# XuZhang1211/PVPUFormer

Measured on AMD Instinct MI355X. Metric: 448x448 images/sec fwd+bwd, ViT-B VPUFormer, higher is better.
Workload: dtype bf16

## Files before the change

include/vpu_hip.h:

```cpp
#ifndef VPU_HIP_H
#define VPU_HIP_H
#include <stdint.h>

#ifdef __cplusplus
extern "C" {
#endif

#define VPU_BF16 0
#define VPU_F32 1

#define VPU_EPI_BIAS 1
#define VPU_EPI_PREACT 2
#define VPU_EPI_GELU 4
#define VPU_EPI_RELU 8
#define VPU_EPI_DGELU 16
#define VPU_EPI_DRELU 32
#define VPU_EPI_RESID 64
#define VPU_EPI_AFFINE 128
#define VPU_EPI_ACCUM 256
#define VPU_EPI_OUT_F32 512
#define VPU_EPI_SAVE_DGELU 1024
#define VPU_EPI_MULAUX 2048

typedef struct vpu_gemm_desc {
// ... 186 lines not shown
    const uint8_t* valid;
    int32_t H, W, r0, r1, c0, c1, mirror, n_obj;
} vpu_box_row;
int vpu_box_prompts_batched(const vpu_box_row* rows, int32_t n_rows, const float* points, int32_t n_batch, int32_t S_h,
                            int32_t S_w, float pred_thresh, uint8_t* masks, int32_t* counts, int32_t* roots, int32_t* slots,
                            int32_t* table, int32_t kmax, int32_t* boxes, int32_t* flag, void* stream);
#define VPU_CROPS_MAX_TILES_AXIS 64
int vpu_crops_gather(const float* in, float* out, const int32_t* y_offsets, const int32_t* x_offsets, int32_t ny, int32_t nx,
                     int32_t C, int32_t H, int32_t W, int32_t ch, int32_t cw, void* stream);
int vpu_crops_blend(const float* probs, float* out, const int32_t* y_offsets, const int32_t* x_offsets, int32_t ny, int32_t nx,
                    int32_t H, int32_t W, int32_t ch, int32_t cw, void* stream);
int vpu_cc_roots(const uint8_t* mask, int32_t* roots, int32_t B, int32_t H, int32_t W, void* stream);
int vpu_cc_table(const int32_t* roots, int32_t* slots, int32_t* table, int32_t kmax, int32_t B, int32_t H, int32_t W,
                 void* stream);

int vpu_disk_maps(const float* points, const int32_t* boxes, float* out, int32_t B, int32_t n, int32_t H, int32_t W,
                  float radius, void* stream);

int vpu_patch_im2col(const float* image4, const float* disks, void* cols, int32_t B, int32_t H, int32_t W, int32_t P,
                     int32_t win_tokens, int32_t dtype, void* stream);
int vpu_patch_im2col_prenorm(const float* image4, const float* disks, void* cols, int32_t B, int32_t H, int32_t W, int32_t P,
                             int32_t win_tokens, int32_t dtype, void* stream);
int vpu_patch_im2col_floor(const float* image4, const float* disks, void* cols, int32_t B, int32_t H, int32_t W, int32_t P,
                           int32_t wside, int32_t prenorm, int32_t dtype, void* stream);
int vpu_window_permute(const void* x, void* y, int32_t B, int32_t g, int32_t wg, int32_t C, int32_t dir, int32_t dtype,
                       void* stream);

int vpu_pixel_shuffle2(const void* in, void* out, const float* bias, int32_t B, int32_t h, int32_t w, int32_t C,
                       int32_t dir, int32_t dtype, void* stream);
int vpu_space_to_depth2_crop(const void* in, void* out, int32_t B, int32_t g, int32_t C, int32_t dir, int32_t dtype,
                             void* stream);
int vpu_pixel_shuffle2_gn_stats(const void* in, void* out, const float* bias, double* stats, int32_t B, int32_t h, int32_t w,
                                int32_t C, int32_t dtype, void* stream);
int vpu_groupnorm_apply(const void* x, const float* w, const float* b, void* y, float* mean, float* rstd, const double* stats,
                        int32_t B, int64_t HW, int32_t C, float eps, int32_t gelu, int32_t dtype, void* stream);
int vpu_pixel_unshuffle2_nblk(int32_t C);
int vpu_pixel_unshuffle2_sums(const void* in, void* out, float* part, int32_t B, int32_t h, int32_t w, int32_t C,
                              int32_t dtype, void* stream);
int vpu_groupnorm_nchunk(void);
int vpu_groupnorm_fwd(const void* x, const float* w, const float* b, void* y, float* mean, float* rstd, double* stats,
                      int32_t B, int64_t HW, int32_t C, float eps, int32_t gelu, int32_t dtype, void* stream);
int vpu_groupnorm_bwd(const void* dy, const void* x, const float* w, const float* b, const float* mean,
                      const float* rstd, void* dx, float* part, double* stats, int32_t B, int64_t HW, int32_t C,
                      int32_t gelu, int32_t dtype, void* stream);
int vpu_bilinear_cl_fwd(const void* in, int32_t ld_in, void* out, int32_t ld_out, int32_t B, int32_t h, int32_t w,
                        int32_t H, int32_t W, int32_t C, int32_t dtype, void* stream);
int vpu_bilinear_cl_bwd(const void* dout, int32_t ld_out, void* din, int32_t ld_in, int32_t B, int32_t h, int32_t w,
                        int32_t H, int32_t W, int32_t C, int32_t dtype, void* stream);
int vpu_upsum_relu(void* io, const void* const* z, const int32_t* h, const int32_t* w, int32_t n, int32_t B, int32_t H,
                   int32_t W, int32_t C, int32_t dtype, void* stream);
int vpu_head_grad_fused(const void* dfn, const void* y, const float* inv, const float* dout, const void* x, const float* w,
                        const float* mask, void* dx, float* part, float* part_b, int64_t rows, int64_t HW, int32_t C,
                        int32_t dtype, void* stream);
int vpu_gate_stats(const void* Q, const void* Kt, float* cg, int32_t* argq, float* sg, int32_t* argc, int32_t B,
                   int32_t nq, int32_t N, int32_t C, int32_t dtype, void* stream);
int vpu_gate_apply(const void* x, const float* cg, const float* sg, void* out, int32_t B, int32_t N, int32_t C,
                   int32_t dtype, void* stream);
int vpu_gate_bwd(const void* dout, const void* x, const float* cg, const int32_t* argq, const float* sg,
                 const int32_t* argc, void* dx, int32_t accum, void* dQ, void* dK, float* part, int32_t B, int32_t nq,
                 int32_t N, int32_t C, int32_t dtype, void* stream);
int vpu_gate_fwd_n(const void* const* Q, const void* const* K, const void* x, void* const* out, float* cg, int32_t* argq,
                   float* sg, int32_t* argc, int32_t n, int32_t B, int32_t nq, int32_t N, int32_t C, int32_t dtype, void* stream);
int vpu_gate_bwd_n(const void* const* dout, const void* x, const float* cg, const int32_t* argq, const float* sg,
                   const int32_t* argc, void* dx, int32_t accum, void* const* dQ, void* const* dK, float* part, int32_t n,
                   int32_t B, int32_t nq, int32_t N, int32_t C, int32_t dtype, void* stream);
int vpu_convseg_fwd(const void* x, const float* w, const float* bias, const float* mask, float* out, int64_t rows,
                    int64_t HW, int32_t C, int32_t dtype, void* stream);
int vpu_convseg_bwd_nblk(int64_t rows);
int vpu_convseg_bwd(const float* dout, const void* x, const float* w, const float* mask, void* dx, int32_t accum,
                    float* part, float* part_b, int64_t rows, int64_t HW, int32_t C, int32_t dtype, void* stream);

int vpu_upsample_ac_fwd(const float* in, float* out, int64_t planes, int32_t h, int32_t w, int32_t H, int32_t W,
                        void* stream);
int vpu_upsample_ac_bwd(const float* dout, float* din, int64_t planes, int32_t h, int32_t w, int32_t H, int32_t W,
                        void* stream);
int vpu_p2cl_fwd_bwd(const float* prob, const float* gt, const int32_t* slot_mask_idx, const float* override_masks,
                     float* loss_part, float* dprob, float grad_scale, int32_t B, int32_t S, int32_t H, int32_t W,
                     void* stream);
int vpu_p2cl_up_nband(int32_t h, int32_t w);
int vpu_p2cl_up_fwd_bwd(const float* sim_low, const float* gt, const int32_t* slot_mask_idx, const float* override_masks,
                        float* loss_part, float* dsim_low, float grad_scale, int32_t B, int32_t S, int32_t h, int32_t w,
                        int32_t H, int32_t W, void* stream);
int vpu_nfl_dice_scratch_doubles(int32_t B);
int vpu_nfl_dice_fwd_bwd(const float* logits, const float* gt, double* sums, float* out, float* dlogits, float w_nfl,
                         float w_dice, int32_t B, int64_t HW, void* stream);

int vpu_loss_finalize(const float* out, const float* part, int32_t B, int32_t npart, double inv_count, float w_nfl,
                      float w_dice, float w_pcl, float iter_weight, float* res, void* stream);

int vpu_adam_step(float* p, const float* g, float* m, float* v, void* shadow_bf16, int64_t n, float lr, float beta1,
                  float beta2, float eps, float weight_decay, int32_t step, float grad_scale, void* stream);
int vpu_adam_step_groups(float* p, const float* g, float* m, float* v, void* shadow_bf16, int64_t n,
                         const int64_t* seg_end, const float* seg_lr, const float* seg_wd, int32_t nseg, float beta1,
                         float beta2, float eps, int32_t decoupled_wd, int32_t step, float grad_scale, void* stream);
int vpu_adam_step_hyper(float* p, const float* g, float* m, float* v, void* shadow_bf16, int64_t n, const float* hyper,
                        const int64_t* seg_end, const float* seg_scale, const float* seg_wd, int32_t nseg, float beta1,
                        float beta2, float eps, float weight_decay, int32_t decoupled_wd, void* stream);


#ifdef __cplusplus
}
#endif
#endif
```

pvpuformer_amd/_lib.py:

```python
import ctypes as C
import os

_HERE = os.path.dirname(os.path.abspath(__file__))
LIB_PATH = os.path.join(_HERE, os.environ.get("VPU_LIB_FILE") or
                        ("libvpu_hip_diag.so" if os.environ.get("VPU_LIB_DIAG", "0") == "1" else "libvpu_hip.so"))

BF16, F32 = 0, 1

EPI_BIAS, EPI_PREACT, EPI_GELU, EPI_RELU, EPI_DGELU, EPI_DRELU = 1, 2, 4, 8, 16, 32
EPI_RESID, EPI_AFFINE, EPI_ACCUM, EPI_OUT_F32 = 64, 128, 256, 512
EPI_SAVE_DGELU, EPI_MULAUX = 1024, 2048


class GemmDesc(C.Structure):
    _fields_ = [
        ("A", C.c_void_p), ("B", C.c_void_p), ("C", C.c_void_p), ("bias", C.c_void_p), ("resid", C.c_void_p),
        ("aux", C.c_void_p), ("preact", C.c_void_p),
        ("M", C.c_int32), ("N", C.c_int32), ("K", C.c_int32),
        ("lda", C.c_int32), ("ldb", C.c_int32), ("ldc", C.c_int32), ("ldr", C.c_int32), ("ldaux", C.c_int32),
        ("batch", C.c_int32), ("inner", C.c_int32),
        ("sAo", C.c_int64), ("sAi", C.c_int64), ("sBo", C.c_int64), ("sBi", C.c_int64),
        ("sCo", C.c_int64), ("sCi", C.c_int64), ("sRo", C.c_int64), ("sRi", C.c_int64),
        ("transA", C.c_int32), ("transB", C.c_int32), ("dtype", C.c_int32), ("flags", C.c_int32),
        ("resid_period", C.c_int32),
# ... 74 lines not shown
    "vpu_add_bcast": [_P, _P, _P, _L, _L, _I, _P],
    "vpu_add4": [_P, _P, _P, _P, _P, _L, _I, _P],
    "vpu_cast2d": [_P, _I, _L, _P, _I, _L, _L, _I, _I, _P],
    "vpu_cast2d_batched": [C.POINTER(CastJob), _I, _P],
    "vpu_fanout_add": [_P, C.POINTER(C.c_void_p), C.POINTER(C.c_int32), _I, _L, _I, _P],
    "vpu_dropout_mask": [_P, _I, _F, C.c_uint64, _P, _P],
    "vpu_fill_f32": [_P, _F, _L, _P],
    "vpu_fill_ranges_f32": [_P, C.POINTER(C.c_int64), C.POINTER(C.c_int64), _I, _F, _P],
    "vpu_debug_spin": [_P, _I, _L, _P],
    "vpu_debug_gemm_times": [_P],
    "vpu_sigmoid_to_channel": [_P, _P, _I, _L, _I, _I, _P],
    "vpu_act_bwd": [_P, _L, _P, _L, _P, _L, _L, _I, _I, _I, _P],
    "vpu_pue_encode": [_P, _P, _P, _P, _P, _I, _I, _I, _I, _I, _I, _P],
    "vpu_cc_roots": [_P, _P, _I, _I, _I, _P],
    "vpu_cc_table": [_P, _P, _P, _I, _I, _I, _I, _P],
    "vpu_edt": [_P, _P, _P, _I, _I, _I, _I, _P],
    "vpu_chamfer5": [_P, _P, _P, _I, _I, _I, _I, _P],
    "vpu_pue_scribble_rows": [_P, _P, _P, _P, _I, _I, _I, _I, _I, _I, _P],
    "vpu_draw_polyline": [_P, _P, _I, _I, _I, _I, _P],
    "vpu_pue_encode_rows": [_P, _P, _P, _P, _P, _P, _P, _I, _I, _I, _I, _I, _I, _P],
    "vpu_draw_prompt_rows": [_P, _P, _P, _P, _P, _I, _I, _I, _I, _I, _P],
    "vpu_mask_bbox": [_P, _F, _P, _I, _P, _I, _I, _I, _P],
    "vpu_masked_argmax": [_P, _P, _P, _I, _I, _I, _P],
    "vpu_error_masks": [_P, _P, _P, _P, _I, _I, _P],
    "vpu_roi_resize_batched": [_P, _I, _P, _I, _I, _I, _I, _P],
    "vpu_roi_paste_batched": [_P, _I, _P, _I, _I, _F, _F, _I, _P],
    "vpu_session_paste_batched": [_P, _I, _P, _I, _I, _F, _F, _I, _I, _P],
    "vpu_annot_compose_batched": [_P, _I, _F, _I, _P],
    "vpu_label_extract": [_P, _P, _P, _I, _I, _I, _P],
    "vpu_runs_count_batched": [_P, _P, _I, _P, _L, _P, _P],
    "vpu_runs_write_batched": [_P, _P, _I, _P, _L, _P, _I, _P],
    "vpu_runs_decode_batched": [_P, _P, _I, _P],
    "vpu_click_keys_batched": [_P, _I, _P, _P, _P, _I, _I, _I, _P],
    "vpu_box_prompts_batched": [_P, _I, _P, _I, _I, _I, _F, _P, _P, _P, _P, _P, _I, _P, _P, _P],
    "vpu_crops_gather": [_P, _P, _P, _P, _I, _I, _I, _I, _I, _I, _I, _P],
    "vpu_crops_blend": [_P, _P, _P, _P, _I, _I, _I, _I, _I, _I, _P],
    "vpu_disk_maps": [_P, _P, _P, _I, _I, _I, _I, _F, _P],
    "vpu_patch_im2col": [_P, _P, _P, _I, _I, _I, _I, _I, _I, _P],
    "vpu_patch_im2col_prenorm": [_P, _P, _P, _I, _I, _I, _I, _I, _I, _P],
    "vpu_patch_im2col_floor": [_P, _P, _P, _I, _I, _I, _I, _I, _I, _I, _P],
    "vpu_window_permute": [_P, _P, _I, _I, _I, _I, _I, _I, _P],
    "vpu_space_to_depth2_crop": [_P, _P, _I, _I, _I, _I, _I, _P],
    "vpu_pixel_shuffle2": [_P, _P, _P, _I, _I, _I, _I, _I, _I, _P],
    "vpu_pixel_shuffle2_gn_stats": [_P, _P, _P, _P, _I, _I, _I, _I, _I, _P],
    "vpu_groupnorm_apply": [_P, _P, _P, _P, _P, _P, _P, _I, _L, _I, _F, _I, _I, _P],
    "vpu_pixel_unshuffle2_nblk": [_I],
    "vpu_pixel_unshuffle2_sums": [_P, _P, _P, _I, _I, _I, _I, _I, _P],
    "vpu_groupnorm_nchunk": [],
    "vpu_groupnorm_fwd": [_P, _P, _P, _P, _P, _P, _P, _I, _L, _I, _F, _I, _I, _P],
    "vpu_groupnorm_bwd": [_P, _P, _P, _P, _P, _P, _P, _P, _P, _I, _L, _I, _I, _I, _P],
    "vpu_bilinear_cl_fwd": [_P, _I, _P, _I, _I, _I, _I, _I, _I, _I, _I, _P],
    "vpu_bilinear_cl_bwd": [_P, _I, _P, _I, _I, _I, _I, _I, _I, _I, _I, _P],
    "vpu_head_grad_fused": [_P, _P, _P, _P, _P, _P, _P, _P, _P, _P, _L, _L, _I, _I, _P],
    "vpu_upsum_relu": [_P, C.POINTER(C.c_void_p), C.POINTER(C.c_int32), C.POINTER(C.c_int32), _I, _I, _I, _I, _I, _I, _P],
    "vpu_gate_stats": [_P, _P, _P, _P, _P, _P, _I, _I, _I, _I, _I, _P],
    "vpu_gate_apply": [_P, _P, _P, _P, _I, _I, _I, _I, _P],
    "vpu_gate_bwd": [_P, _P, _P, _P, _P, _P, _P, _I, _P, _P, _P, _I, _I, _I, _I, _I, _P],
    "vpu_gate_fwd_n": [C.POINTER(C.c_void_p), C.POINTER(C.c_void_p), _P, C.POINTER(C.c_void_p), _P, _P, _P, _P, _I, _I, _I, _I, _I, _I, _P],
    "vpu_gate_bwd_n": [C.POINTER(C.c_void_p), _P, _P, _P, _P, _P, _P, _I, C.POINTER(C.c_void_p), C.POINTER(C.c_void_p), _P, _I, _I, _I,
                       _I, _I, _I, _P],
    "vpu_convseg_fwd": [_P, _P, _P, _P, _P, _L, _L, _I, _I, _P],
    "vpu_convseg_bwd_nblk": [_L],
    "vpu_convseg_bwd": [_P, _P, _P, _P, _P, _I, _P, _P, _L, _L, _I, _I, _P],
    "vpu_upsample_ac_fwd": [_P, _P, _L, _I, _I, _I, _I, _P],
    "vpu_upsample_ac_bwd": [_P, _P, _L, _I, _I, _I, _I, _P],
    "vpu_p2cl_fwd_bwd": [_P, _P, _P, _P, _P, _P, _F, _I, _I, _I, _I, _P],
    "vpu_p2cl_up_nband": [_I, _I],
    "vpu_p2cl_up_fwd_bwd": [_P, _P, _P, _P, _P, _P, _F, _I, _I, _I, _I, _I, _I, _P],
    "vpu_nfl_dice_scratch_doubles": [_I],
    "vpu_nfl_dice_fwd_bwd": [_P, _P, _P, _P, _P, _F, _F, _I, _L, _P],
    "vpu_loss_finalize": [_P, _P, _I, _I, C.c_double, _F, _F, _F, _F, _P, _P],
    "vpu_adam_step": [_P, _P, _P, _P, _P, _L, _F, _F, _F, _F, _F, _I, _F, _P],
    "vpu_adam_step_groups": [_P, _P, _P, _P, _P, _L, _P, _P, _P, _I, _F, _F, _F, _I, _I, _F, _P],
    "vpu_adam_step_hyper": [_P, _P, _P, _P, _P, _L, _P, _P, _P, _P, _I, _F, _F, _F, _F, _I, _P],
    "vpu_gemm_set_option": [C.c_char_p, _I],
    "vpu_gemm_get_option": [C.c_char_p, C.POINTER(C.c_int32)],
    "vpu_gemm_last_kernel": [],
    "vpu_attn_last_kernel": [],
    "vpu_attn_set_option": [C.c_char_p, _I],
    "vpu_gemm_grouped": [C.POINTER(GemmDesc), _I, _P],
    "vpu_last_error": [],
    "vpu_abi_version": [],
}
_RET = {"vpu_last_error": C.c_char_p, "vpu_gemm_last_kernel": C.c_char_p, "vpu_attn_last_kernel": C.c_char_p}

_lib = None


class VpuError(RuntimeError):
    pass


def load():
    global _lib
    if _lib is not None:
        return _lib
    if not os.path.exists(LIB_PATH):
        raise VpuError(f"{LIB_PATH} not found: build it with pvpuformer_amd/csrc/build.sh "
                       f"(or `python -c 'import __graft_entry__ as g; g.build()'`). There is no CPU fallback.")
    import torch
    lib = C.CDLL(LIB_PATH)
    for name, argtypes in SIGNATURES.items():
        fn = getattr(lib, name)
        fn.argtypes = argtypes
        fn.restype = _RET.get(name, C.c_int)
    _lib = lib
# ... 10 lines not shown
```

pvpuformer_amd/engine.py:

```python
import contextlib
import math
import os
from collections import OrderedDict
from types import SimpleNamespace

import numpy as np
import torch

from . import ops
from ._lib import (BF16, F32, EPI_BIAS, EPI_PREACT, EPI_GELU, EPI_RELU, EPI_DGELU, EPI_DRELU, EPI_RESID, EPI_AFFINE,
                   EPI_ACCUM, EPI_OUT_F32, EPI_SAVE_DGELU, EPI_MULAUX)


class Tape:
    __slots__ = ("fns", "out_grads", "done", "sim_low", "lane")

    def __init__(self):
        self.fns = []
        self.out_grads = [None, None, None]
        self.done = False
        self.sim_low = None
        self.lane = None

    def append(self, fn):
# ... 58 lines not shown


def check_square(H, W):
    if H != W:
        raise ValueError(f"input {H}x{W}: only square inputs are supported (the reference's neck takes h = w = sqrt(HW))")


class Engine:
    def __init__(self, cfg, dtype="bf16", device="cuda"):
        self.cfg = dict(cfg)
        self.dt = BF16 if dtype in ("bf16", BF16) else F32
        self.td = torch.bfloat16 if self.dt == BF16 else torch.float32
        self.dev = torch.device(device)
        c = self.cfg
        self.D, self.P, self.img = c["embed_dim"], c["patch"], c["img"]
        self.g, _, self.wside = window_geometry(self.img, self.P)
        self.NT = self.g * self.g
        self.heads = c["num_heads"]
        self.depth = c["depth"]
        self.group = 6 if self.depth == 12 else self.depth // 4
        self.nmax = c["num_max_points"]
        self.E = 2 * self.img + 3
        self.Epad = _rup(self.E, 8)
        self.C = c["head_channels"]
        self.out_dims = tuple(c["out_dims"])
        self.names = None
        self.tape = Tape()
        self.last_tape = None
        self.params = []
        self.norm_radius = float(c.get("norm_radius", 5))
        self.training = False
        self.shadow_valid = False
        self._const_ready = False
        self.use_flash = True
        self.use_side = os.environ.get("VPU_WGRAD_STREAM", "0") == "1"
        self.side = None
        self.fuse_ln_pe = True
        self.group_wgrad = True
        self.ride_wgrad = True
        self.wgrad_fill = 0.8
        hid = self.D * c["mlp_ratio"]
        blk = sum(((n + 255) // 256) * ((k + 127) // 128) for n, k in ((3 * self.D, self.D), (self.D, self.D), (hid, self.D), (self.D, hid)))
        pk = os.environ.get("VPU_WGRAD_PACK", "")
        k3 = ops.gemm_get_option("k3")
        k4_default = (k3 & 8) != 0
        self.pack_wgrad = pk == "1" or (pk != "0" and (blk < 0.95 * 256 or k4_default))
        self.k3_wgrad = (k3 & 1) != 0
        self.k4_wgrad = (k3 & 8) != 0
        self.wgrad_round = 256 if (self.k4_wgrad or not self.k3_wgrad) else 512
        self.wgrad_tn = 256 if self.k4_wgrad else 128
        self.unify_wgrad = True
        self.lazy_zero = True
        self.xattn_split = max(1, int(os.environ.get("VPU_XATTN_SPLIT", "1")))
        self.neck_lanes = int(os.environ.get("VPU_NECK_LANES", "0"))
        self._tok_stream = None
        self._in_lanes = False
        self.dist_colsum = True
        self._pack_seen, self._pack_total = {}, {}
        self._pending_reports, self._reporting = [], False
        self.group_tiles = 256
        self.split_wgrad = True
        self._wq = []
        self._csq = []
        self._gq = []
        self._gq_out = set()
        self._frozen = set()
        self._token_rows = 0
        self.grad_ready_hook = None
        self.report_lag = max(1, int(os.environ.get("VPU_DIST_REPORT_LAG", "2")))

    def bind(self, named_params):
        self.names = OrderedDict()
        off = 0
        for n, p in named_params.items():
            self.names[n] = (off, tuple(p.shape), p.numel())
            off = _rup(off + p.numel(), 8)
        self.total = off
        self.flat = torch.zeros(off, device=self.dev, dtype=torch.float32)
        self.gflat = torch.zeros(off, device=self.dev, dtype=torch.float32)
        self.params = []
        for n, p in named_params.items():
            o, shape, numel = self.names[n]
            view = self.flat[o:o + numel].view(shape)
            view.copy_(p.data)
            p.data = view
            p.grad = self.gflat[o:o + numel].view(shape)
            self.params.append((p, o, shape, numel))
        self.shadow = torch.zeros(off, device=self.dev, dtype=torch.bfloat16) if self.dt == BF16 else None
        self._lazy = set()
        self._lazy_names, self._lazy_ranges = self._lazy_plan()
        D, P = self.D, self.P
        self.k3p = _rup(3 * P * P, 8)
        self.w_patch = torch.zeros(D, 2 * self.k3p, device=self.dev, dtype=self.td)
        self.b_patch = torch.zeros(D, device=self.dev, dtype=torch.float32)
        self.w_lin1p = torch.zeros(2048, self.Epad, device=self.dev, dtype=self.td)
        self.pos_win = torch.zeros(self.NT, D, device=self.dev, dtype=self.td)
        self._pos_cache, self._kpe_cache, self._regrid_cache = {}, {}, {}
        self.shadow_valid = False
        if not self._const_ready:
            self.kpe = pos2d_table(D, self.g, self.g).to(self.dev).to(self.td)
            self.lut = torch.from_numpy(click_lut()).to(self.dev)
            self._const_ready = True

    def W(self, name):
        o = self.names[name][0]
        return (self.shadow, o) if self.dt == BF16 else (self.flat, o)
# ... 940 lines not shown

    def _head(self, cx, feats, q_out, drop_mask, materialize_aux):
        B, H, W_, nq, o, tape = cx.B, cx.H, cx.W, cx.nq, self.out_dims, self.tape
        Cc, Hs = self.C, 4 * cx.g
        HW4 = Hs * Hs
        wf, ldf = self.W("head.fusion_conv.conv.weight"), 4 * Cc
        gf = self.G("head.fusion_conv.conv.weight")
        relu_done, ymask = [False], [[False] for _ in range(4)]
        ys, zs = [], []
        for i in range(4):
            f, s = feats[i]
            ys.append(self.linear(f, f"head.convs.{i}.conv.weight", f"head.convs.{i}.conv.bias", B * s * s, Cc, o[i],
                                  act="relu", pre_masked=ymask[i]))
        fused = Var(self._new(B * HW4, Cc))
        ops.gemm(ys[0].t, wf, fused.t, B * HW4, Cc, Cc, Cc, ldf, Cc, self.dt, flags=EPI_BIAS,
                 bias=self.Pm("head.fusion_conv.conv.bias"))
        for i in (1, 2, 3):
            s = feats[i][1]
            z = self._new(B * s * s, Cc)
            ops.gemm(ys[i].t, (wf[0], wf[1] + i * Cc), z, B * s * s, Cc, Cc, Cc, ldf, Cc, self.dt)
            zs.append((z, s, s))
        ops.upsum_relu(fused.t, zs, B, Hs, Hs, Cc, self.dt)
        if cx.training:
            def bwd_fusion():
                if fused.g is None:
                    return
                if relu_done[0]:
                    dt_ = fused.g
                else:
                    dt_ = self._new(B * HW4, Cc)
                    ops.act_bwd(fused.g, Cc, fused.t, Cc, dt_, Cc, B * HW4, Cc, 0, self.dt)
                self._wgrad(dt_, Cc, ys[0].t, Cc, gf, Cc, Cc, B * HW4, ldc=ldf, bias="head.fusion_conv.conv.bias")
                fuse_mask = self.dt == BF16
                mk = dict(flags=EPI_DRELU, ldaux=Cc) if fuse_mask else {}
                self._dgrad(dt_, Cc, wf, ldf, ys[0], B * HW4, Cc, Cc, **(dict(mk, aux=ys[0].t) if fuse_mask else {}))
                ymask[0][0] = fuse_mask
                for i in (1, 2, 3):
                    s = feats[i][1]
                    dz = self._new(B * s * s, Cc)
                    ops.bilinear_cl_bwd(dt_, Cc, dz, Cc, B, s, s, Hs, Hs, Cc, self.dt)
                    self._wgrad(dz, Cc, ys[i].t, Cc, (gf[0], gf[1] + i * Cc), Cc, Cc, B * s * s, ldc=ldf)
                    self._dgrad(dz, Cc, (wf[0], wf[1] + i * Cc), ldf, ys[i], B * s * s, Cc, Cc,
                                **(dict(mk, aux=ys[i].t) if fuse_mask else {}))
                    ymask[i][0] = fuse_mask
            self.tape.append(bwd_fusion)
        seg = self._new(B * HW4, dtype=torch.float32)
        ops.convseg_fwd(fused.t, self.Pm("head.conv_seg.weight"), self.Pm("head.conv_seg.bias"), drop_mask, seg,
                        B * HW4, HW4, Cc)
        dm = self.cfg["head_d_model"]
        query = self.mlp(q_out, "head.ffn_layer.lin1", "head.ffn_layer.lin2", B * nq, dm, 2 * dm, Cc, "relu")
        qn, fn = Var(torch.empty_like(query.t)), Var(torch.empty_like(fused.t))
        inv_q, inv_f = self._new(B * nq, dtype=torch.float32), self._new(B * HW4, dtype=torch.float32)
        ops.l2norm_fwd(query.t, qn.t, inv_q, B * nq, Cc)
        ops.l2norm_fwd(fused.t, fn.t, inv_f, B * HW4, Cc)
        sim = self._new(B, nq, HW4, dtype=torch.float32)
        ops.gemm(qn.t, fn.t, sim, nq, HW4, Cc, Cc, Cc, HW4, self.dt, flags=EPI_OUT_F32 | EPI_AFFINE, post_mul=0.5,
                 post_add=0.5, batch=B, inner=1, sA=(nq * Cc, 0), sB=(HW4 * Cc, 0), sC=(nq * HW4, 0))
        if cx.taps is not None:
            cx.taps["seg_lowres"] = seg.view(B, 1, Hs, Hs)
            cx.taps["sim_lowres"] = sim.view(B, nq, Hs, Hs)
            cx.taps["fused"] = fused.t
        inst = self._new(B, 1, H, W_, dtype=torch.float32)
        ops.upsample_ac_fwd(seg, inst, B, Hs, Hs, H, W_)
        aux = None
        self.sim_low = sim.view(B, nq, Hs, Hs)
        if materialize_aux:
            aux = self._new(B, nq, H, W_, dtype=torch.float32)
            ops.upsample_ac_fwd(sim, aux, B * nq, Hs, Hs, H, W_)
        tape.sim_low = self.sim_low
        if cx.training:
            def bwd_head():
                d_inst, d_aux, d_sim_low = tape.out_grads
                if d_aux is not None or d_sim_low is not None:
                    if d_sim_low is not None:
                        dsim = d_sim_low.view(B, nq, HW4)
                    else:
                        dsim = self._new(B, nq, HW4, dtype=torch.float32)
                        ops.upsample_ac_bwd(d_aux, dsim, B * nq, Hs, Hs, H, W_)
                    if self.dt == BF16:
                        dsim_t = self._new(B, nq, HW4)
                        ops.cast2d(dsim, HW4, dsim_t, HW4, B * nq, HW4)
                    else:
                        dsim_t = dsim
                    qn.g, fn.g = torch.empty_like(qn.t), torch.empty_like(fn.t)
                    ops.gemm(dsim_t, fn.t, qn.g, nq, Cc, HW4, HW4, Cc, Cc, self.dt, transB=True, alpha=0.5, batch=B,
                             inner=1, sA=(nq * HW4, 0), sB=(HW4 * Cc, 0), sC=(nq * Cc, 0))
                    ops.gemm(dsim_t, qn.t, fn.g, HW4, Cc, nq, HW4, Cc, Cc, self.dt, transA=True, transB=True, alpha=0.5,
                             batch=B, inner=1, sA=(nq * HW4, 0), sB=(nq * Cc, 0), sC=(HW4 * Cc, 0))
                    query.g = torch.empty_like(query.t)
                    ops.l2norm_bwd(qn.g, qn.t, inv_q, query.g, B * nq, Cc)
                    one_pass = d_inst is not None and self.dt == BF16 and Cc in (64, 128, 256, 512)
                    if not one_pass:
                        fused.g = torch.empty_like(fused.t)
                        ops.l2norm_bwd(fn.g, fn.t, inv_f, fused.g, B * HW4, Cc)
                if d_inst is not None:
                    dseg = self._new(B * HW4, dtype=torch.float32)
                    ops.upsample_ac_bwd(d_inst, dseg, B, Hs, Hs, H, W_)
                    nb = ops.convseg_bwd_nblk(B * HW4)
                    part, part_b = self._new(nb, Cc, dtype=torch.float32), self._new(nb, dtype=torch.float32)
                    if (d_aux is not None or d_sim_low is not None) and one_pass:
                        fused.g = torch.empty_like(fused.t)
                        ops.head_grad_fused(fn.g, fn.t, inv_f, dseg, fused.t, self.Pm("head.conv_seg.weight"), drop_mask,
                                            fused.g, part, part_b, B * HW4, HW4, Cc)
                    else:
                        accum = fused.g is not None
                        if not accum:
                            fused.g = torch.empty_like(fused.t)
                        self._writable(fused.g)
                        ops.convseg_bwd(dseg, fused.t, self.Pm("head.conv_seg.weight"), drop_mask, fused.g, int(accum) | 2, part,
                                        part_b, B * HW4, HW4, Cc)
                    relu_done[0] = True
                    self._csq.append((part, self.G("head.conv_seg.weight"), nb, Cc))
                    self._csq.append((part_b, self.G("head.conv_seg.bias"), nb, 1))
            self.tape.append(bwd_head)
        return inst, aux

    def _mark_ready(self, first_name, next_name):
        lo = self.names[first_name][0]
        hi = self.total if next_name is None else self.names[next_name][0]

        def marker():
            if self.ride_wgrad and self.group_wgrad and self.dt == BF16 and not self.use_side:
                self.flush_wgrads(0)
                if self.grad_ready_hook is not None:
                    for k in sorted({e[3] for e in self._wq if e[3] > 2048} - {self._token_rows}):
                        self.flush_wgrads(k)
                    self._pending_reports.append((lo, hi))
                    self._report_ready()
                    if len(self._pending_reports) > self.report_lag:
                        lo0, hi0 = self._pending_reports[0]
                        off_of = lambda t: t[1] if isinstance(t, tuple) else None
                        late = [e for e in self._wq
                                if any(off_of(t) is None or lo0 <= off_of(t) < hi0 for t in self._targets(e))]
                        if late:
                            self.flush_wgrads(entries=late)
                return
            self.flush_wgrads()
            if self.grad_ready_hook is not None:
                self._pending_reports.append((lo, hi))
                self._report_ready()
        self.tape.append(marker)
# ... 260 lines not shown
```

pvpuformer_amd/ops.py:

```python
import ctypes as C

import torch

from . import _lib
from ._lib import (BF16, F32, EPI_BIAS, EPI_PREACT, EPI_GELU, EPI_RELU, EPI_DGELU, EPI_DRELU, EPI_RESID, EPI_AFFINE,
                   EPI_ACCUM, EPI_OUT_F32, EPI_SAVE_DGELU, EPI_MULAUX, GemmDesc)

TORCH_DTYPE = {BF16: torch.bfloat16, F32: torch.float32}


def code_of(t):
    if isinstance(t, tuple):
        t = t[0]
    if t.dtype == torch.bfloat16:
        return BF16
    if t.dtype == torch.float32:
        return F32
    raise TypeError(f"unsupported dtype {t.dtype}")


_raw_stream = getattr(torch._C, "_cuda_getCurrentRawStream", None)
_cur_device = getattr(torch._C, "_cuda_getDevice", None)


# ... 561 lines not shown
    n = len(maps)
    zp = (C.c_void_p * 3)(*[ptr(m[0]) for m in maps])
    hs = (C.c_int32 * 3)(*[m[1] for m in maps])
    ws = (C.c_int32 * 3)(*[m[2] for m in maps])
    _lib.call("vpu_upsum_relu", ptr(io), zp, hs, ws, n, B, H, W, Cdim, dtype, _stream())


def gate_stats(Q, Kt, cg, argq, sg, argc, B, nq, N, Cdim):
    _lib.call("vpu_gate_stats", ptr(Q), ptr(Kt), ptr(cg), ptr(argq), ptr(sg), ptr(argc), B, nq, N, Cdim, code_of(Q),
              _stream())


def gate_apply(x, cg, sg, out, B, N, Cdim):
    _lib.call("vpu_gate_apply", ptr(x), ptr(cg), ptr(sg), ptr(out), B, N, Cdim, code_of(x), _stream())


def gate_bwd(dout, x, cg, argq, sg, argc, dx, accum, dQ, dK, part, B, nq, N, Cdim):
    _lib.call("vpu_gate_bwd", ptr(dout), ptr(x), ptr(cg), ptr(argq), ptr(sg), ptr(argc), ptr(dx), int(accum), ptr(dQ),
              ptr(dK), ptr(part), B, nq, N, Cdim, code_of(x), _stream())


def _ptr_array(ts):
    return (C.c_void_p * len(ts))(*[ptr(t) for t in ts])


def gate_fwd_n(Qs, Ks, x, outs, cg, argq, sg, argc, B, nq, N, Cdim):
    _lib.call("vpu_gate_fwd_n", _ptr_array(Qs), _ptr_array(Ks), ptr(x), _ptr_array(outs), ptr(cg), ptr(argq), ptr(sg), ptr(argc),
              len(Qs), B, nq, N, Cdim, code_of(x), _stream())


def gate_bwd_n(douts, x, cg, argq, sg, argc, dx, accum, dQs, dKs, part, B, nq, N, Cdim):
    _lib.call("vpu_gate_bwd_n", _ptr_array(douts), ptr(x), ptr(cg), ptr(argq), ptr(sg), ptr(argc), ptr(dx), int(accum),
              _ptr_array(dQs), _ptr_array(dKs), ptr(part), len(douts), B, nq, N, Cdim, code_of(x), _stream())


def convseg_fwd(x, w, bias, mask, out, rows, HW, Cdim):
    _lib.call("vpu_convseg_fwd", ptr(x), ptr(w), ptr(bias), ptr(mask), ptr(out), rows, HW, Cdim, code_of(x), _stream())


def convseg_bwd_nblk(rows):
    return _lib.load().vpu_convseg_bwd_nblk(rows)


def convseg_bwd(dout, x, w, mask, dx, accum, part, part_b, rows, HW, Cdim):
    _lib.call("vpu_convseg_bwd", ptr(dout), ptr(x), ptr(w), ptr(mask), ptr(dx), int(accum), ptr(part), ptr(part_b),
              rows, HW, Cdim, code_of(x), _stream())


def head_grad_fused(dfn, y, inv, dout, x, w, mask, dx, part, part_b, rows, HW, Cdim):
    _lib.call("vpu_head_grad_fused", ptr(dfn), ptr(y), ptr(inv), ptr(dout), ptr(x), ptr(w), ptr(mask), ptr(dx), ptr(part),
              ptr(part_b), rows, HW, Cdim, code_of(x), _stream())


def upsample_ac_fwd(inp, out, planes, h, w, H, W):
    _lib.call("vpu_upsample_ac_fwd", ptr(inp), ptr(out), planes, h, w, H, W, _stream())


def upsample_ac_bwd(dout, din, planes, h, w, H, W):
    _lib.call("vpu_upsample_ac_bwd", ptr(dout), ptr(din), planes, h, w, H, W, _stream())


def p2cl_fwd_bwd(prob, gt, slot_idx, override, loss_part, dprob, grad_scale, B, S, H, W):
    _lib.call("vpu_p2cl_fwd_bwd", ptr(prob), ptr(gt), ptr(slot_idx), ptr(override), ptr(loss_part), ptr(dprob),
              grad_scale, B, S, H, W, _stream())


def p2cl_up_fwd_bwd(sim_low, gt, slot_idx, override, loss_part, dsim_low, grad_scale, B, S, h, w, H, W):
    nband = _lib.load().vpu_p2cl_up_nband(h, w)
    bands = torch.empty(B * S, nband, device=sim_low.device, dtype=torch.float32)
    _lib.call("vpu_p2cl_up_fwd_bwd", ptr(sim_low), ptr(gt), ptr(slot_idx), ptr(override), ptr(bands), ptr(dsim_low),
              grad_scale, B, S, h, w, H, W, _stream())
    if loss_part is None:
        return bands
    torch.sum(bands, dim=1, out=loss_part.view(B * S))
    return loss_part


def nfl_dice_fwd_bwd(logits, gt, sums, out, dlogits, w_nfl, w_dice, B, HW):
    if sums is None:
        sums = torch.empty(_lib.load().vpu_nfl_dice_scratch_doubles(B), device=logits.device, dtype=torch.float64)
    _lib.call("vpu_nfl_dice_fwd_bwd", ptr(logits), ptr(gt), ptr(sums), ptr(out), ptr(dlogits), w_nfl, w_dice, B, HW,
              _stream())


def loss_finalize(out, part, B, npart, inv_count, w_nfl, w_dice, w_pcl, iter_weight, res):
    _lib.call("vpu_loss_finalize", ptr(out), ptr(part), B, npart, float(inv_count), w_nfl, w_dice, w_pcl, iter_weight,
              ptr(res), _stream())


def adam_step_groups(p, g, m, v, shadow, n, seg_end, seg_lr, seg_wd, nseg, b1, b2, eps, decoupled, step, grad_scale=1.0):
    _lib.call("vpu_adam_step_groups", ptr(p), ptr(g), ptr(m), ptr(v), ptr(shadow), n, ptr(seg_end), ptr(seg_lr),
              ptr(seg_wd), nseg, b1, b2, eps, int(decoupled), step, grad_scale, _stream())


def adam_step_hyper(p, g, m, v, shadow, n, hyper, seg_end, seg_scale, seg_wd, nseg, b1, b2, eps, wd, decoupled):
    _lib.call("vpu_adam_step_hyper", ptr(p), ptr(g), ptr(m), ptr(v), ptr(shadow), n, ptr(hyper), ptr(seg_end),
              ptr(seg_scale), ptr(seg_wd), nseg, b1, b2, eps, wd, int(decoupled), _stream())


def adam_step(p, g, m, v, shadow, n, lr, b1, b2, eps, wd, step, grad_scale=1.0):
    _lib.call("vpu_adam_step", ptr(p), ptr(g), ptr(m), ptr(v), ptr(shadow), n, lr, b1, b2, eps, wd, step, grad_scale,
              _stream())
```

Measured before the change: 976.0.

## Fuse L2-norm with query-similarity GEMM and add dedicated similarity backward kernels

```diff
diff --git a/include/vpu_hip.h b/include/vpu_hip.h
--- a/include/vpu_hip.h
+++ b/include/vpu_hip.h
@@ -262,6 +262,11 @@
 int vpu_head_grad_fused(const void* dfn, const void* y, const float* inv, const float* dout, const void* x, const float* w,
                         const float* mask, void* dx, float* part, float* part_b, int64_t rows, int64_t HW, int32_t C,
                         int32_t dtype, void* stream);
+int vpu_sim_fwd(const void* fused, const void* qn, void* fn, float* inv_f, float* sim, int32_t B, int32_t nq, int64_t HW,
+                int32_t C, int32_t max_blocks, void* stream);
+int vpu_sim_bwd_parts(int32_t B, int64_t HW);
+int vpu_sim_bwd(const float* d_sim, const void* qn, const void* fn, void* d_fn, void* d_qn, float* part, int32_t parts,
+                int32_t B, int32_t nq, int64_t HW, int32_t C, int32_t max_blocks, void* stream);
 int vpu_gate_stats(const void* Q, const void* Kt, float* cg, int32_t* argq, float* sg, int32_t* argc, int32_t B,
                    int32_t nq, int32_t N, int32_t C, int32_t dtype, void* stream);
 int vpu_gate_apply(const void* x, const float* cg, const float* sg, void* out, int32_t B, int32_t N, int32_t C,
diff --git a/pvpuformer_amd/_lib.py b/pvpuformer_amd/_lib.py
--- a/pvpuformer_amd/_lib.py
+++ b/pvpuformer_amd/_lib.py
@@ -150,6 +150,9 @@
     "vpu_bilinear_cl_fwd": [_P, _I, _P, _I, _I, _I, _I, _I, _I, _I, _I, _P],
     "vpu_bilinear_cl_bwd": [_P, _I, _P, _I, _I, _I, _I, _I, _I, _I, _I, _P],
     "vpu_head_grad_fused": [_P, _P, _P, _P, _P, _P, _P, _P, _P, _P, _L, _L, _I, _I, _P],
+    "vpu_sim_fwd": [_P, _P, _P, _P, _P, _I, _I, _L, _I, _I, _P],
+    "vpu_sim_bwd_parts": [_I, _L],
+    "vpu_sim_bwd": [_P, _P, _P, _P, _P, _P, _I, _I, _I, _L, _I, _I, _P],
     "vpu_upsum_relu": [_P, C.POINTER(C.c_void_p), C.POINTER(C.c_int32), C.POINTER(C.c_int32), _I, _I, _I, _I, _I, _I, _P],
     "vpu_gate_stats": [_P, _P, _P, _P, _P, _P, _I, _I, _I, _I, _I, _P],
     "vpu_gate_apply": [_P, _P, _P, _P, _I, _I, _I, _I, _P],
diff --git a/pvpuformer_amd/csrc/sim.hip b/pvpuformer_amd/csrc/sim.hip
--- /dev/null
+++ b/pvpuformer_amd/csrc/sim.hip
@@ -0,0 +1,357 @@
+#include <stdlib.h>
+#include "vpu_common.h"
+#include "../../include/vpu_hip.h"
+
+#define ST reinterpret_cast<hipStream_t>(stream)
+
+namespace {
+
+typedef __attribute__((address_space(3))) s16x4_t* lds_s16x4_ptr;
+constexpr int SIM_MAXQ = 48;
+constexpr int SIM_OCC = 2;
+
+__device__ __forceinline__ uint4 ldg16(const bf16_t* p) { return *reinterpret_cast<const uint4*>(p); }
+
+template <int NKS>
+__global__ __launch_bounds__(256, SIM_OCC) void sim_fwd_kernel(const bf16_t* __restrict__ x, const bf16_t* __restrict__ qn,
+                                                      bf16_t* __restrict__ fn, float* __restrict__ inv,
+                                                      float* __restrict__ sim, int nq, int HW) {
+    constexpr int C = NKS * 32, QLD = C * 2 + 16;
+    __shared__ __attribute__((aligned(16))) char lq[SIM_MAXQ * QLD];
+    const int b = blockIdx.y, tid = threadIdx.x, lane = tid & 63, n = lane & 15, g = lane >> 4;
+    for (int c = tid; c < SIM_MAXQ * (C / 8); c += 256) {
+        const int q = c / (C / 8), ch = c - q * (C / 8);
+        uint4 v = make_uint4(0, 0, 0, 0);
+        if (q < nq) v = ldg16(qn + ((int64_t)b * nq + q) * C + ch * 8);
+        *reinterpret_cast<uint4*>(lq + q * QLD + ch * 16) = v;
+    }
+    __syncthreads();
+    const int ntiles = (HW + 15) >> 4, tstride = gridDim.x * 4;
+    const bf16_t* xb = x + (int64_t)b * HW * C;
+    bf16_t* fb = fn + (int64_t)b * HW * C;
+    float* ib = inv + (int64_t)b * HW;
+    float* sb = sim + (int64_t)b * nq * HW;
+    int tile = blockIdx.x * 4 + (tid >> 6);
+    uint4 cur[NKS], nxt[NKS];
+#pragma unroll
+    for (int ks = 0; ks < NKS; ++ks) {
+        cur[ks] = make_uint4(0, 0, 0, 0);
+        if (tile < ntiles && tile * 16 + n < HW) cur[ks] = ldg16(xb + (int64_t)(tile * 16 + n) * C + ks * 32 + g * 8);
+    }
+    for (; tile < ntiles; tile += tstride) {
+        const int row = tile * 16 + n, nrow = row + tstride * 16;
+#pragma unroll
+        for (int ks = 0; ks < NKS; ++ks) {
+            nxt[ks] = make_uint4(0, 0, 0, 0);
+            if (nrow < HW) nxt[ks] = ldg16(xb + (int64_t)nrow * C + ks * 32 + g * 8);
+        }
+        float tot;
+        if constexpr (NKS == 1) {
+            const bf16x8_t r = __builtin_bit_cast(bf16x8_t, cur[0]);
+            float e[8];
+#pragma unroll
+            for (int j = 0; j < 8; ++j) {
+                const float v = (float)r[j];
+                e[j] = v * v;
+                e[j] += __shfl_xor(e[j], 32, 64);
+                e[j] += __shfl_xor(e[j], 16, 64);
+            }
+#pragma unroll
+            for (int o = 4; o > 0; o >>= 1) {
+#pragma unroll
+                for (int i = 0; i < o; ++i) e[i] = e[i] + e[i ^ o];
+            }
+            tot = e[0];
+        } else {
+            float s[NKS];
+#pragma unroll
+            for (int ks = 0; ks < NKS; ++ks) {
+                const bf16x8_t r = __builtin_bit_cast(bf16x8_t, cur[ks]);
+                s[ks] = 0.f;
+#pragma unroll
+                for (int j = 0; j < 8; ++j) { const float v = (float)r[j]; s[ks] += v * v; }
+            }
+#pragma unroll
+            for (int o = NKS >> 1; o > 0; o >>= 1) {
+#pragma unroll
+                for (int i = 0; i < o; ++i) s[i] = s[i] + s[i ^ o];
+            }
+            tot = s[0];
+            tot += __shfl_xor(tot, 32, 64);
+            tot += __shfl_xor(tot, 16, 64);
+        }
+        const float iv = 1.0f / fmaxf(sqrtf(tot), 1e-12f);
+        bf16x8_t bf[NKS];
+#pragma unroll
+        for (int ks = 0; ks < NKS; ++ks) {
+            const bf16x8_t r = __builtin_bit_cast(bf16x8_t, cur[ks]);
+#pragma unroll
+            for (int j = 0; j < 8; ++j) { float v = (float)r[j]; v *= iv; bf[ks][j] = (bf16_t)v; }
+        }
+        if (row < HW) {
+            if (g == 0) ib[row] = iv;
+#pragma unroll
+            for (int ks = 0; ks < NKS; ++ks)
+                *reinterpret_cast<bf16x8_t*>(fb + (int64_t)row * C + ks * 32 + g * 8) = bf[ks];
+        }
+        f32x4_t acc[3];
+#pragma unroll
+        for (int t = 0; t < 3; ++t) acc[t] = f32x4_t{0.f, 0.f, 0.f, 0.f};
+#pragma unroll
+        for (int ks = 0; ks < NKS; ++ks) {
+#pragma unroll
+            for (int t = 0; t < 3; ++t) {
+                const bf16x8_t a = __builtin_bit_cast(
+                    bf16x8_t, *reinterpret_cast<const uint4*>(lq + (t * 16 + n) * QLD + ks * 64 + g * 16));
+                acc[t] = __builtin_amdgcn_mfma_f32_16x16x32_bf16(a, bf[ks], acc[t], 0, 0, 0);
+            }
+        }
+        if (row < HW) {
+#pragma unroll
+            for (int t = 0; t < 3; ++t) {
+#pragma unroll
+                for (int r = 0; r < 4; ++r) {
+                    const int q = t * 16 + 4 * g + r;
+                    if (q < nq) sb[(int64_t)q * HW + row] = 0.5f * acc[t][r] + 0.5f;
+                }
+            }
+        }
+#pragma unroll
+        for (int ks = 0; ks < NKS; ++ks) cur[ks] = nxt[ks];
+    }
+}
+
+template <int NKS>
+__global__ __launch_bounds__(256, SIM_OCC) void sim_dfn_kernel(const float* __restrict__ dsim, const bf16_t* __restrict__ qn,
+                                                      bf16_t* __restrict__ dfn, int nq, int HW) {
+    constexpr int C = NKS * 32, TLD = 64 * 2 + 16;
+    __shared__ __attribute__((aligned(16))) char lt[C * TLD];
+    const int b = blockIdx.y, tid = threadIdx.x, lane = tid & 63, n = lane & 15, g = lane >> 4;
+    for (int c = tid; c < 64 * (C / 8); c += 256) {
+        const int q = c / (C / 8), ch = c - q * (C / 8);
+        uint4 v = make_uint4(0, 0, 0, 0);
+        if (q < nq) v = ldg16(qn + ((int64_t)b * nq + q) * C + ch * 8);
+        const bf16x8_t r = __builtin_bit_cast(bf16x8_t, v);
+#pragma unroll
+        for (int j = 0; j < 8; ++j) *reinterpret_cast<bf16_t*>(lt + (ch * 8 + j) * TLD + q * 2) = r[j];
+    }
+    __syncthreads();
+    const int ntiles = (HW + 15) >> 4, tstride = gridDim.x * 4;
+    const float* db = dsim + (int64_t)b * nq * HW;
+    bf16_t* ob = dfn + (int64_t)b * HW * C;
+    int tile = blockIdx.x * 4 + (tid >> 6);
+    float cur[16], nxt[16];
+#pragma unroll
+    for (int e = 0; e < 16; ++e) {
+        const int q = (e >> 3) * 32 + g * 8 + (e & 7);
+        cur[e] = 0.f;
+        if (tile < ntiles && tile * 16 + n < HW && q < nq) cur[e] = db[(int64_t)q * HW + tile * 16 + n];
+    }
+    for (; tile < ntiles; tile += tstride) {
+        const int row = tile * 16 + n, nrow = row + tstride * 16;
+#pragma unroll
+        for (int e = 0; e < 16; ++e) {
+            const int q = (e >> 3) * 32 + g * 8 + (e & 7);
+            nxt[e] = 0.f;
+            if (nrow < HW && q < nq) nxt[e] = db[(int64_t)q * HW + nrow];
+        }
+        bf16x8_t bf[2];
+#pragma unroll
+        for (int e = 0; e < 16; ++e) bf[e >> 3][e & 7] = (bf16_t)cur[e];
+#pragma unroll
+        for (int p = 0; p < NKS; ++p) {
+            f32x4_t acc[2];
+#pragma unroll
+            for (int u = 0; u < 2; ++u) {
+                acc[u] = f32x4_t{0.f, 0.f, 0.f, 0.f};
+                const int c = 32 * p + 8 * (n >> 2) + 4 * u + (n & 3);
+#pragma unroll
+                for (int ks = 0; ks < 2; ++ks) {
+                    const bf16x8_t a = __builtin_bit_cast(
+                        bf16x8_t, *reinterpret_cast<const uint4*>(lt + c * TLD + ks * 64 + g * 16));
+                    acc[u] = __builtin_amdgcn_mfma_f32_16x16x32_bf16(a, bf[ks], acc[u], 0, 0, 0);
+                }
+            }
+            if (row < HW) {
+                bf16x8_t o;
+#pragma unroll
+                for (int r = 0; r < 4; ++r) { o[r] = (bf16_t)(0.5f * acc[0][r]); o[4 + r] = (bf16_t)(0.5f * acc[1][r]); }
+                *reinterpret_cast<bf16x8_t*>(ob + (int64_t)row * C + 32 * p + 8 * g) = o;
+            }
+        }
+#pragma unroll
+        for (int e = 0; e < 16; ++e) cur[e] = nxt[e];
+    }
+}
+
+template <int NKS>
+__global__ __launch_bounds__(256) void sim_dqn_kernel(const float* __restrict__ dsim, const bf16_t* __restrict__ fn,
+                                                      float* __restrict__ part, int nq, int HW, int steps_per_part) {
+    constexpr int C = NKS * 32, RLD = C * 2 + 32, CPR = C / 8, NLD = (32 * CPR + 255) / 256;
+    constexpr int CW = C / 4 < 16 ? 16 : C / 4, NCT = CW / 16;
+    __shared__ __attribute__((aligned(16))) char lf[32 * RLD];
+    const int b = blockIdx.y, tid = threadIdx.x, lane = tid & 63, wave = tid >> 6, n = lane & 15, g = lane >> 4;
+    const int nsteps = (HW + 31) >> 5;
+    const int s0 = blockIdx.x * steps_per_part, s1 = min(nsteps, s0 + steps_per_part);
+    const bf16_t* fb = fn + (int64_t)b * HW * C;
+    const float* db = dsim + (int64_t)b * nq * HW;
+    const bool vec4 = (HW & 3) == 0 && (reinterpret_cast<uintptr_t>(dsim) & 15) == 0;
+    f32x4_t acc[3][NCT];
+#pragma unroll
+    for (int t = 0; t < 3; ++t)
+#pragma unroll
+        for (int ct = 0; ct < NCT; ++ct) acc[t][ct] = f32x4_t{0.f, 0.f, 0.f, 0.f};
+    uint4 stage[NLD];
+    auto fetch = [&](int step) {
+#pragma unroll
+        for (int i = 0; i < NLD; ++i) {
+            const int c = tid + i * 256, r = c / CPR, ch = c - r * CPR;
+            stage[i] = make_uint4(0, 0, 0, 0);
+            if (c < 32 * CPR && step < s1 && step * 32 + r < HW) stage[i] = ldg16(fb + (int64_t)(step * 32 + r) * C + ch * 8);
+        }
+    };
+    fetch(s0);
+    for (int step = s0; step < s1; ++step) {
+        __syncthreads();
+#pragma unroll
+        for (int i = 0; i < NLD; ++i) {
+            const int c = tid + i * 256, r = c / CPR, ch = c - r * CPR;
+            if (c < 32 * CPR) *reinterpret_cast<uint4*>(lf + r * RLD + ch * 16) = stage[i];
+        }
+        const int row0 = step * 32 + 4 * g;
+        bf16x8_t af[3];
+#pragma unroll
+        for (int t = 0; t < 3; ++t) {
+            const int q = t * 16 + n;
+            float v[8] = {0.f, 0.f, 0.f, 0.f, 0.f, 0.f, 0.f, 0.f};
+            if (q < nq) {
+                const float* src = db + (int64_t)q * HW;
+                if (vec4) {
+                    if (row0 < HW) { const float4 a = *reinterpret_cast<const float4*>(src + row0); v[0] = a.x; v[1] = a.y; v[2] = a.z; v[3] = a.w; }
+                    if (row0 + 16 < HW) { const float4 a = *reinterpret_cast<const float4*>(src + row0 + 16); v[4] = a.x; v[5] = a.y; v[6] = a.z; v[7] = a.w; }
+                } else {
+#pragma unroll
+                    for (int j = 0; j < 4; ++j) {
+                        if (row0 + j < HW) v[j] = src[row0 + j];
+                        if (row0 + 16 + j < HW) v[4 + j] = src[row0 + 16 + j];
+                    }
+                }
+            }
+#pragma unroll
+            for (int j = 0; j < 8; ++j) af[t][j] = (bf16_t)v[j];
+        }
+        fetch(step + 1);
+        __syncthreads();
+        const int qq = n >> 2, pp = n & 3;
+        if (wave * CW >= C) continue;
+#pragma unroll
+        for (int ct = 0; ct < NCT; ++ct) {
+            const int col = wave * CW + ct * 16 + 4 * pp;
+            const s16x4_t lo = __builtin_amdgcn_ds_read_tr16_b64_v4i16((lds_s16x4_ptr)(lf + (4 * g + qq) * RLD + col * 2));
+            const s16x4_t hi = __builtin_amdgcn_ds_read_tr16_b64_v4i16((lds_s16x4_ptr)(lf + (16 + 4 * g + qq) * RLD + col * 2));
+            s16x8_t v;
+            v[0] = lo[0]; v[1] = lo[1]; v[2] = lo[2]; v[3] = lo[3];
+            v[4] = hi[0]; v[5] = hi[1]; v[6] = hi[2]; v[7] = hi[3];
+            const bf16x8_t bfr = __builtin_bit_cast(bf16x8_t, v);
+#pragma unroll
+            for (int t = 0; t < 3; ++t) acc[t][ct] = __builtin_amdgcn_mfma_f32_16x16x32_bf16(af[t], bfr, acc[t][ct], 0, 0, 0);
+        }
+    }
+    if (wave * CW >= C) return;
+    float* pb = part + ((int64_t)b * gridDim.x + blockIdx.x) * SIM_MAXQ * C;
+#pragma unroll
+    for (int t = 0; t < 3; ++t)
+#pragma unroll
+        for (int ct = 0; ct < NCT; ++ct)
+#pragma unroll
+            for (int r = 0; r < 4; ++r) pb[(t * 16 + 4 * g + r) * C + wave * CW + ct * 16 + n] = acc[t][ct][r];
+}
+
+__global__ __launch_bounds__(256) void sim_dqn_reduce_kernel(const float* __restrict__ part, bf16_t* __restrict__ dqn,
+                                                             int parts, int nq, int C, int64_t total4) {
+    const int64_t i = (int64_t)blockIdx.x * 256 + threadIdx.x;
+    if (i >= total4) return;
+    const int c4 = C >> 2;
+    const int64_t bq = i / c4;
+    const int c = (int)(i - bq * c4) * 4, b = (int)(bq / nq), q = (int)(bq - (int64_t)b * nq);
+    const float* src = part + ((int64_t)b * parts * SIM_MAXQ + q) * C + c;
+    float4 s = make_float4(0.f, 0.f, 0.f, 0.f);
+    for (int p = 0; p < parts; ++p) {
+        const float4 v = *reinterpret_cast<const float4*>(src + (int64_t)p * SIM_MAXQ * C);
+        s.x += v.x; s.y += v.y; s.z += v.z; s.w += v.w;
+    }
+    bf16_t* o = dqn + bq * C + c;
+    o[0] = (bf16_t)(0.5f * s.x); o[1] = (bf16_t)(0.5f * s.y); o[2] = (bf16_t)(0.5f * s.z); o[3] = (bf16_t)(0.5f * s.w);
+}
+
+bool sim_args_ok(const char* who, int B, int nq, int64_t HW, int C, int max_blocks) {
+    if (B < 1 || B > 65535 || nq < 1 || nq > SIM_MAXQ || HW < 1 || HW > (1 << 26) || !(C == 32 || C == 64 || C == 128 || C == 256) ||
+        max_blocks < 0) {
+        vpu_set_error(who);
+        return false;
+    }
+    return true;
+}
+bool aligned16(const void* a, const void* b, const void* c = nullptr) {
+    return ((reinterpret_cast<uintptr_t>(a) | reinterpret_cast<uintptr_t>(b) | reinterpret_cast<uintptr_t>(c)) & 15) == 0;
+}
+int sim_blocks(int B, int64_t HW, int max_blocks) {
+    const int64_t tiles = (HW + 15) / 16;
+    int64_t g = (tiles + 3) / 4;
+    const int64_t cap = max_blocks > 0 ? max_blocks : (512 + B - 1) / B;
+    if (g > cap) g = cap;
+    return (int)(g < 1 ? 1 : g);
+}
+
+}
+
+#define DISPATCH_C(C, ...)                           \
+    if ((C) == 256) { constexpr int NKS = 8; __VA_ARGS__ } \
+    else if ((C) == 128) { constexpr int NKS = 4; __VA_ARGS__ } \
+    else if ((C) == 64) { constexpr int NKS = 2; __VA_ARGS__ } \
+    else { constexpr int NKS = 1; __VA_ARGS__ }
+
+extern "C" int vpu_sim_fwd(const void* fused, const void* qn, void* fn, float* inv_f, float* sim, int32_t B, int32_t nq,
+                           int64_t HW, int32_t C, int32_t max_blocks, void* stream) {
+    vpu_clear_stale_error();
+    if (!sim_args_ok("sim_fwd: bf16, 1 <= nq <= 48, C in {32,64,128,256}, B <= 65535, HW <= 2^26", B, nq, HW, C, max_blocks))
+        return VPU_ERR_ARG;
+    if (!fused || !qn || !fn || !inv_f || !sim) { vpu_set_error("sim_fwd: null operand"); return VPU_ERR_ARG; }
+    if (!aligned16(fused, qn, fn)) { vpu_set_error("sim_fwd: fused, qn and fn must be 16-byte aligned"); return VPU_ERR_ALIGN; }
+    const dim3 grid(sim_blocks(B, HW, max_blocks), B);
+    DISPATCH_C(C, sim_fwd_kernel<NKS><<<grid, 256, 0, ST>>>((const bf16_t*)fused, (const bf16_t*)qn, (bf16_t*)fn, inv_f, sim,
+                                                            nq, (int)HW);)
+    return vpu_check_launch("vpu_sim_fwd");
+}
+
+extern "C" int vpu_sim_bwd_parts(int32_t B, int64_t HW) {
+    const int64_t steps = (HW + 31) / 32;
+    int64_t p = (steps + 7) / 8;
+    const int64_t cap = B >= 8 ? 32 : 64;
+    if (p > cap) p = cap;
+    return (int)(p < 1 ? 1 : p);
+}
+
+extern "C" int vpu_sim_bwd(const float* d_sim, const void* qn, const void* fn, void* d_fn, void* d_qn, float* part,
+                           int32_t parts, int32_t B, int32_t nq, int64_t HW, int32_t C, int32_t max_blocks, void* stream) {
+    vpu_clear_stale_error();
+    if (!sim_args_ok("sim_bwd: bf16, 1 <= nq <= 48, C in {32,64,128,256}, B <= 65535, HW <= 2^26", B, nq, HW, C, max_blocks))
+        return VPU_ERR_ARG;
+    if (!d_sim || !qn || !fn || !d_fn || !d_qn || !part || parts < 1 || parts > 65535) {
+        vpu_set_error("sim_bwd: null operand, or parts outside [1, 65535]");
+        return VPU_ERR_ARG;
+    }
+    if (!aligned16(qn, fn, d_fn) || !aligned16(part, part) || (reinterpret_cast<uintptr_t>(d_qn) & 7) != 0) {
+        vpu_set_error("sim_bwd: qn, fn, d_fn and part must be 16-byte aligned, d_qn 8-byte aligned");
+        return VPU_ERR_ALIGN;
+    }
+    const dim3 grid(sim_blocks(B, HW, max_blocks), B);
+    DISPATCH_C(C, sim_dfn_kernel<NKS><<<grid, 256, 0, ST>>>(d_sim, (const bf16_t*)qn, (bf16_t*)d_fn, nq, (int)HW);)
+    if (int rc = vpu_check_launch("vpu_sim_bwd (d fn)")) return rc;
+    const int nsteps = (int)((HW + 31) / 32), spp = (nsteps + parts - 1) / parts;
+    DISPATCH_C(C, sim_dqn_kernel<NKS><<<dim3(parts, B), 256, 0, ST>>>(d_sim, (const bf16_t*)fn, part, nq, (int)HW, spp);)
+    if (int rc = vpu_check_launch("vpu_sim_bwd (d qn)")) return rc;
+    const int64_t total4 = (int64_t)B * nq * (C / 4);
+    sim_dqn_reduce_kernel<<<(unsigned)((total4 + 255) / 256), 256, 0, ST>>>(part, (bf16_t*)d_qn, parts, nq, C, total4);
+    return vpu_check_launch("vpu_sim_bwd (reduce)");
+}
diff --git a/pvpuformer_amd/engine.py b/pvpuformer_amd/engine.py
--- a/pvpuformer_amd/engine.py
+++ b/pvpuformer_amd/engine.py
@@ -134,6 +134,7 @@
         self.unify_wgrad = True
         self.lazy_zero = True
         self.xattn_split = max(1, int(os.environ.get("VPU_XATTN_SPLIT", "1")))
+        self.sim_stream = True
         self.neck_lanes = int(os.environ.get("VPU_NECK_LANES", "0"))
         self._tok_stream = None
         self._in_lanes = False
@@ -1180,10 +1181,14 @@
         qn, fn = Var(torch.empty_like(query.t)), Var(torch.empty_like(fused.t))
         inv_q, inv_f = self._new(B * nq, dtype=torch.float32), self._new(B * HW4, dtype=torch.float32)
         ops.l2norm_fwd(query.t, qn.t, inv_q, B * nq, Cc)
-        ops.l2norm_fwd(fused.t, fn.t, inv_f, B * HW4, Cc)
         sim = self._new(B, nq, HW4, dtype=torch.float32)
-        ops.gemm(qn.t, fn.t, sim, nq, HW4, Cc, Cc, Cc, HW4, self.dt, flags=EPI_OUT_F32 | EPI_AFFINE, post_mul=0.5,
-                 post_add=0.5, batch=B, inner=1, sA=(nq * Cc, 0), sB=(HW4 * Cc, 0), sC=(nq * HW4, 0))
+        sim_stream = self.sim_stream and self.dt == BF16 and Cc in (32, 64, 128, 256) and nq <= 48
+        if sim_stream:
+            ops.sim_fwd(fused.t, qn.t, fn.t, inv_f, sim, B, nq, HW4, Cc)
+        else:
+            ops.l2norm_fwd(fused.t, fn.t, inv_f, B * HW4, Cc)
+            ops.gemm(qn.t, fn.t, sim, nq, HW4, Cc, Cc, Cc, HW4, self.dt, flags=EPI_OUT_F32 | EPI_AFFINE, post_mul=0.5,
+                     post_add=0.5, batch=B, inner=1, sA=(nq * Cc, 0), sB=(HW4 * Cc, 0), sC=(nq * HW4, 0))
         if cx.taps is not None:
             cx.taps["seg_lowres"] = seg.view(B, 1, Hs, Hs)
             cx.taps["sim_lowres"] = sim.view(B, nq, Hs, Hs)
@@ -1205,16 +1210,20 @@
                     else:
                         dsim = self._new(B, nq, HW4, dtype=torch.float32)
                         ops.upsample_ac_bwd(d_aux, dsim, B * nq, Hs, Hs, H, W_)
-                    if self.dt == BF16:
-                        dsim_t = self._new(B, nq, HW4)
-                        ops.cast2d(dsim, HW4, dsim_t, HW4, B * nq, HW4)
+                    qn.g, fn.g = torch.empty_like(qn.t), torch.empty_like(fn.t)
+                    if sim_stream:
+                        part = self._new(B, ops.sim_bwd_parts(B, HW4), 48, Cc, dtype=torch.float32)
+                        ops.sim_bwd(dsim, qn.t, fn.t, fn.g, qn.g, part, B, nq, HW4, Cc)
                     else:
-                        dsim_t = dsim
-                    qn.g, fn.g = torch.empty_like(qn.t), torch.empty_like(fn.t)
-                    ops.gemm(dsim_t, fn.t, qn.g, nq, Cc, HW4, HW4, Cc, Cc, self.dt, transB=True, alpha=0.5, batch=B,
-                             inner=1, sA=(nq * HW4, 0), sB=(HW4 * Cc, 0), sC=(nq * Cc, 0))
-                    ops.gemm(dsim_t, qn.t, fn.g, HW4, Cc, nq, HW4, Cc, Cc, self.dt, transA=True, transB=True, alpha=0.5,
-                             batch=B, inner=1, sA=(nq * HW4, 0), sB=(nq * Cc, 0), sC=(HW4 * Cc, 0))
+                        if self.dt == BF16:
+                            dsim_t = self._new(B, nq, HW4)
+                            ops.cast2d(dsim, HW4, dsim_t, HW4, B * nq, HW4)
+                        else:
+                            dsim_t = dsim
+                        ops.gemm(dsim_t, fn.t, qn.g, nq, Cc, HW4, HW4, Cc, Cc, self.dt, transB=True, alpha=0.5, batch=B,
+                                 inner=1, sA=(nq * HW4, 0), sB=(HW4 * Cc, 0), sC=(nq * Cc, 0))
+                        ops.gemm(dsim_t, qn.t, fn.g, HW4, Cc, nq, HW4, Cc, Cc, self.dt, transA=True, transB=True,
+                                 alpha=0.5, batch=B, inner=1, sA=(nq * HW4, 0), sB=(nq * Cc, 0), sC=(HW4 * Cc, 0))
                     query.g = torch.empty_like(query.t)
                     ops.l2norm_bwd(qn.g, qn.t, inv_q, query.g, B * nq, Cc)
                     one_pass = d_inst is not None and self.dt == BF16 and Cc in (64, 128, 256, 512)
diff --git a/pvpuformer_amd/ops.py b/pvpuformer_amd/ops.py
--- a/pvpuformer_amd/ops.py
+++ b/pvpuformer_amd/ops.py
@@ -637,6 +637,19 @@
               ptr(part_b), rows, HW, Cdim, code_of(x), _stream())
 
 
+def sim_fwd(fused, qn, fn, inv_f, sim, B, nq, HW, Cdim, max_blocks=0):
+    _lib.call("vpu_sim_fwd", ptr(fused), ptr(qn), ptr(fn), ptr(inv_f), ptr(sim), B, nq, HW, Cdim, max_blocks, _stream())
+
+
+def sim_bwd_parts(B, HW):
+    return _lib.load().vpu_sim_bwd_parts(B, HW)
+
+
+def sim_bwd(d_sim, qn, fn, d_fn, d_qn, part, B, nq, HW, Cdim, max_blocks=0):
+    _lib.call("vpu_sim_bwd", ptr(d_sim), ptr(qn), ptr(fn), ptr(d_fn), ptr(d_qn), ptr(part), part.shape[1], B, nq, HW, Cdim,
+              max_blocks, _stream())
+
+
 def upsample_ac_fwd(inp, out, planes, h, w, H, W):
     _lib.call("vpu_upsample_ac_fwd", ptr(inp), ptr(out), planes, h, w, H, W, _stream())
 
```

Result: no change. 978.4, median of 5 (+0.2%).
